# multiplefish/VPLines-SLAM

Measured on AMD Instinct MI355X. Metric: sliding-window BA solves/sec (10 KF, 200 pts + 80 lines, 5 iters), higher is better.
Workload: dtype f64

## Files before the change

### vplines-slam_amd/csrc/ba_step.h

```cpp
#pragma once
#include "ba_common.h"
#include "ba_solve.h"

namespace vpl {

constexpr int SCHUR_THREADS = 256;
constexpr int CHOL_THREADS = 256;
constexpr int BACK_THREADS = 256;

__device__ __forceinline__ void lds_ticket_wait(int* t, int seq) {
  while (__hip_atomic_load(t, __ATOMIC_RELAXED, __HIP_MEMORY_SCOPE_WORKGROUP) != seq) __builtin_amdgcn_s_sleep(1);
  __builtin_amdgcn_fence(__ATOMIC_ACQUIRE, "workgroup", "local");
}
__device__ __forceinline__ void lds_ticket_pass(int* t, int seq, int lane) {
  __builtin_amdgcn_fence(__ATOMIC_RELEASE, "workgroup", "local");
  if (lane == 0) __hip_atomic_store(t, seq + 1, __ATOMIC_RELAXED, __HIP_MEMORY_SCOPE_WORKGROUP);
}

__device__ __forceinline__ int compact2vis(int c, int s, int WS) {
  if (c < WS - 6) { const int v = 6 * s + c; return v < 66 ? v : -1; }
  if (c < WS) return 66 + (c - (WS - 6));
  return c < WS + 2 ? 72 + (c - WS) : -1;
}

// ... 453 lines not shown
      const int k0 = __builtin_amdgcn_readlane(wrow, __builtin_amdgcn_readfirstlane(1 + 3 * ch));
      const int k1 = __builtin_amdgcn_readlane(wrow, __builtin_amdgcn_readfirstlane(2 + 3 * ch));
      const int seq = __builtin_amdgcn_readlane(wrow, __builtin_amdgcn_readfirstlane(3 + 3 * ch));
      nent += k1 - k0;
      if (MIXED && (fetch(k0).x & 64)) {
        SchurWide A;
        A.etab = etab; A.Wp = Wp; A.Wl = Wl; A.WS = WS; A.lC = lC; A.lS = lS; A.lE = lE; A.lG = lG; A.pS = pS; A.pE = pE; A.pG = pG;
        A.Cacc = Cacc; A.tick = tick;
        schur_wide_chunk(A, k0, k1, seq);
        continue;
      }
      double raw0[NTC][4], raw1[NTC][4], raw2[NTC][4];
      constexpr int NPF = 3;
      load_raw(fetch(k0), raw0);
      load_raw(fetch(min(k0 + 1, k1 - 1)), raw1);
      load_raw(fetch(min(k0 + 2, k1 - 1)), raw2);
      const int gcur = fetch(k0).x;
      auto step = [&](int k, double (&rw)[NTC][4]) {
        const int4 e = fetch(k);
#ifdef VPL_STAMPS
        const long long ts0 = __builtin_readcyclecounter();
#endif
        double x[NTC][4];
        transform(e, rw, x);
#ifdef VPL_STAMPS
        const long long ts1 = __builtin_readcyclecounter();
        st_xf += ts1 - ts0;
#endif
        load_raw(fetch(min(k + NPF, k1 - 1)), rw);
#ifdef VPL_STAMPS
        const long long ts2 = __builtin_readcyclecounter();
        st_ld += ts2 - ts1;
#endif
        const bool isl = (e.x & 32) != 0;
#pragma unroll
        for (int a = 0; a < 4; ++a) {
          if (a == 0 || isl) {
            int t = 0;
#pragma unroll
            for (int ta = 0; ta < NTC; ++ta)
#pragma unroll
              for (int tb = 0; tb <= ta; ++tb, ++t) acc[t] = __builtin_amdgcn_mfma_f64_16x16x4f64(x[ta][a], x[tb][a], acc[t], 0, 0, 0);
          }
        }
#ifdef VPL_STAMPS
        st_mf += __builtin_readcyclecounter() - ts2;
#endif
      };
#pragma unroll 1
      for (int kb = k0; kb < k1; kb += NPF) {
        step(kb, raw0);
        if (kb + 1 < k1) step(kb + 1, raw1);
        if (kb + 2 < k1) step(kb + 2, raw2);
      }
      flush(gcur, seq);
    }
#ifdef VPL_STAMPS
    if (lane == 0 && wv < 2) {
      long long* dg_ = B.dbg + (size_t)w * 64 + 30 + 6 * wv;
      dg_[0] = st_xf; dg_[1] = st_ld; dg_[2] = st_mf; dg_[3] = st_flush; dg_[4] = st_wait; dg_[5] = nent;
    }
#endif
  }
  __syncthreads();
  VPL_STAMP(B, w, 3);
  for (int b = tid; b < NV; b += T) qq += 2.0 * Cacc[(NV + 1) * CSQ_LD + b] * uc[vis2cam(b)];
  double* sacc = B.sacc + (size_t)w * SACC_N;
  for (int i = tid; i < SACC_N; i += T) {
    int a, b;
    tri_decode(i, a, b);
    sacc[i] = Cacc[a * CSQ_LD + b];
  }
  a1 = block_sum(a1, red);
  q = block_sum(q, red);
  qq = block_sum(qq, red);
  if (tid == 0) {
    tr->a1 = a1;
    tr->alpha = a1 / (q + qq);
    if (flag[0]) B.path[w] = 2;
  }
  VPL_STAMP(B, w, 4);
}

template <int NTC>
__global__ __launch_bounds__(SCHUR_THREADS, 2) void k_schur(DevBatch B) {
  extern __shared__ double sm[];
  if (blockIdx.x == 0 && threadIdx.x == 0) { B.ord_cnt[2 * ((B.ord_it + 1) & 1)] = 0; B.ord_cnt[2 * ((B.ord_it + 1) & 1) + 1] = 0; }
  schur_body<NTC>(B, ordered_window(B), sm);
}
__global__ __launch_bounds__(SCHUR_THREADS, 2) void k_schur_mixed(DevBatch B) {
  extern __shared__ double sm[];
  if (blockIdx.x == 0 && threadIdx.x == 0) { B.ord_cnt[2 * ((B.ord_it + 1) & 1)] = 0; B.ord_cnt[2 * ((B.ord_it + 1) & 1) + 1] = 0; }
  schur_body<3, true>(B, ordered_window(B), sm);
}
inline size_t schur_smem(int maxP, int maxL, int ntc = 5) {
  const int r1 = std::max(4 * maxP + 28 * maxL, (int)CSQ_N);
  const int maxKS = maxP / 4 + maxL + NF + 2;
  return (size_t)(r1 + 3 * maxP + 22 * maxL + 176 + 24) * sizeof(double) + (size_t)(8 + 4 * maxKS + ntc * (ntc + 1) / 2 * 256) * sizeof(int);
}

constexpr int DN = 90;
constexpr int DNT = 6;
constexpr int DNAP = DNT * (DNT + 1) / 2 * 256;
constexpr int XLD = 80;
constexpr int CHOL_MIN_WAVES = 2;
constexpr int XROWS_A = 36, XROWS_B = 48;
__device__ __forceinline__ constexpr int xcol(int ch, int J) { return ch == 0 ? 16 * (J > 3 ? J - 1 : J) : 16 * (J - 1); }
__device__ __forceinline__ constexpr int tile_row(int t) { return t < 1 ? 0 : t < 3 ? 1 : t < 6 ? 2 : t < 10 ? 3 : t < 15 ? 4 : 5; }

__device__ __forceinline__ int chain_frame(int ch, int b) { return ch == 0 ? 1 + b : 10 - b; }
__device__ __forceinline__ int chain_col(int ch, int b, int lane) {
  if (lane < 18) {
    const int ds = (b & 1) ? 9 : 0;
    const int f = chain_frame(ch, b);
    const int fr = (lane >= ds && lane < ds + 9) ? f : (ch == 0 ? f + 1 : f - 1);
    return 15 * fr + 6 + (lane < 9 ? lane : lane - 9);
  }
  if (ch == 0) {
    if (lane < 27) return 6 + (lane - 18);
    if (lane < 63) return 15 * ((lane - 27) / 6) + (lane - 27) % 6;
    return NC;
  }
  if (lane < 54) return 15 * (5 + (lane - 18) / 6) + (lane - 18) % 6;
  return lane == 54 ? NC : -1;
}
__device__ __forceinline__ int cam2dense(int c) {
  if (c < 0) return -1;
  if (c == NC) return DN;
  const int v = cam2vis(c);
  if (v >= 0) return v;
  if (c < 15) return 72 + (c - 6);
  return (c >= 81 && c < 90) ? c : -1;
}
__device__ __forceinline__ int dense2cam(int d) { return d < NV ? vis2cam(d) : (d < 81 ? 6 + (d - 72) : d); }
__device__ __forceinline__ int chain_dense(int ch, int lane) {
  if (lane < 18) {
    const bool s5 = ch == 0 ? lane < 9 : lane >= 9;
    return s5 ? 81 + (lane < 9 ? lane : lane - 9) : -1;
  }
  return cam2dense(chain_col(ch, 0, lane));
}

__device__ __forceinline__ void chol_body(const DevBatch& B, const int w, double* sm) {
  const int tid = threadIdx.x, T = CHOL_THREADS;
  const int lane = tid & 63, wv = ((tid >> 6) + ((blockIdx.x >> 8) & 1) * 2) & 3;
  TrState* tr = &B.tr[w];
  if (tr->status != 0 || tr->reuse != 0 || B.path[w] != 0) return;
  count_active(B, 1);
  constexpr int REG = (XROWS_A + XROWS_B) * XLD > DNAP ? (XROWS_A + XROWS_B) * XLD : DNAP;
  double* XA = sm;
  double* XBm = sm + XROWS_A * XLD;
  double* S = sm;
  double* scv = sm + REG;
  double* dgv = scv + 176;
  double* ycam = dgv + 176;
  double* yv = ycam + 176;
  double* isd = yv + 96;
  double* Linv = isd + 96;
  double* red = Linv + 256;
  int* flag = (int*)(red + 24);
  double* rsL = (double*)(flag + 8);

  const size_t fb = (size_t)w * B.nfull;
  const double* gscale = B.scale + fb;
  const double* gdiag = B.diag + fb;
  const double* ggrad = B.grad + fb;
  double* ggn = B.gn + fb;
  const double* Hcc = B.Hcc + (size_t)w * NCP;
  const double* gc = B.gc + (size_t)w * NC;
  const double* sacc = B.sacc + (size_t)w * SACC_N;
  const double mu = tr->mu;
  for (int c = tid; c < 176; c += T) { scv[c] = c < NC ? gscale[c] : 0.0; dgv[c] = c < NC ? gdiag[c] : 1.0; ycam[c] = 0.0; }
  if (tid < 4) flag[tid] = 0;
  for (int i = tid; i < (XROWS_A + XROWS_B) * XLD; i += T) sm[i] = 0.0;
  __syncthreads();
  VPL_STAMP(B, w, 8);

  double U[45];
#pragma unroll
  for (int i = 0; i < 45; ++i) U[i] = 0.0;
#define Xs(b, k) U[9 * (b) + (k)]
  if (wv < 2) {
    const int ch = wv, nblk = ch == 0 ? 4 : 5;
    double* Xout = ch == 0 ? XA : XBm;
    const int xd = chain_dense(ch, lane);
    const int xp = xd < 0 ? -1 : xcol(ch, xd >> 4) + (xd & 15);
    bool bad = false;
    auto load_strip = [&](int b, double (&raw)[9]) {
      const int col = chain_col(ch, b, lane);
      const int f = chain_frame(ch, b);
#pragma unroll
      for (int i = 0; i < 9; ++i) {
        const int r = 15 * f + 6 + i;
        raw[i] = 0.0;
        if (col == NC) raw[i] = gc[r];
        else if (col >= 0) raw[i] = Hcc[col > r ? tri(col, r) : tri(r, col)];
      }
    };
    double rawn[9];
    load_strip(0, rawn);
#pragma unroll
    for (int b = 0; b < 5; ++b) {
      if (b < nblk) {
        const int ds = (b & 1) ? 9 : 0, ns = 9 - ds;
        const int col = chain_col(ch, b, lane);
        const int f = chain_frame(ch, b);
        double R[9];
        {
          const double scol = col == NC ? 1.0 : (col >= 0 ? scv[col] : 0.0);
#pragma unroll
          for (int i = 0; i < 9; ++i) {
            const int r = 15 * f + 6 + i;
            R[i] = rawn[i] * (scv[r] * scol);
            if (col == r) R[i] += mu * dgv[r] * dgv[r];
          }
        }
        if (b + 1 < nblk) load_strip(b + 1, rawn);
        if (b > 0) {
          const bool fresh = lane >= ns && lane < ns + 9;
#pragma unroll
          for (int k = 0; k < 9; ++k) {
            const double xk = fresh ? 0.0 : Xs(b - 1, k);
#pragma unroll
            for (int i = 0; i < 9; ++i) R[i] -= readlane_f64(Xs(b - 1, k), ds + i) * xk;
          }
        }
        double piv[9];
#pragma unroll
        for (int k = 0; k < 9; ++k) {
          const double pk = readlane_f64(R[k], ds + k);
          piv[k] = pk;
          if (!(pk > 0.0)) bad = true;
          double rinv = __builtin_amdgcn_rcp(pk);
          rinv = fma(rinv, fma(-pk, rinv, 1.0), rinv);
          rinv = fma(rinv, fma(-pk, rinv, 1.0), rinv);
          const double fj = R[k] * rinv;
#pragma unroll
          for (int i = k + 1; i < 9; ++i) R[i] -= readlane_f64(R[i], ds + k) * fj;
        }
        const bool dcol = cam2dense(col) >= 0;
#pragma unroll
        for (int k = 0; k < 9; ++k) {
          double rs = __builtin_amdgcn_rsq(piv[k]);
          rs = rs * fma(-0.5 * piv[k] * rs, rs, 1.5);
          rs = rs * fma(-0.5 * piv[k] * rs, rs, 1.5);
          if (lane == 0) rsL[(5 * ch + b) * 9 + k] = rs;
          const double xv = R[k] * rs;
          Xs(b, k) = col >= 0 ? xv : 0.0;
          if (xp >= 0) Xout[(9 * b + k) * XLD + xp] = dcol ? xv : 0.0;
        }
        __builtin_amdgcn_fence(__ATOMIC_RELEASE, "workgroup");
        if (lane == 0) __hip_atomic_store(&flag[1 + ch], b + 1, __ATOMIC_RELAXED, __HIP_MEMORY_SCOPE_WORKGROUP);
      }
    }
    if (bad && lane == 0) flag[0] = 1;
  } else {
    const int m = lane & 15, kk = lane >> 4;
    auto h0 = [&](int r, int c) -> double {
      if (r < c) { const int t = r; r = c; c = t; }
      if (r > DN || c == DN) return r == c ? 1.0 : 0.0;
      const int cc = dense2cam(c);
      if (r == DN) return (gc[cc] - (c < NV ? sacc[tri(NV, c)] : 0.0)) * scv[cc];
      const int cr = dense2cam(r);
      double v = Hcc[cr >= cc ? tri(cr, cc) : tri(cc, cr)];
      if (r < NV) v -= sacc[tri(r, c)];
      v *= scv[cr] * scv[cc];
      if (r == c) v += mu * dgv[cr] * dgv[cr];
      return v;
    };
    const int p = __builtin_amdgcn_readfirstlane(wv - 2);
    v4d hs[11], acc[11];
#pragma unroll
    for (int i = 0; i < 11; ++i) acc[i] = v4d{0, 0, 0, 0};
    int have = 0;
#pragma unroll 1
    for (int ks = 0; ks < XROWS_A / 4; ++ks) {
      const int need = min(4, (4 * ks + 3) / 9 + 1);
      while (have < need) {
        have = __hip_atomic_load(&flag[1], __ATOMIC_RELAXED, __HIP_MEMORY_SCOPE_WORKGROUP);
        if (have >= need) __builtin_amdgcn_fence(__ATOMIC_ACQUIRE, "workgroup");
      }
      const double* row = XA + (4 * ks + kk) * XLD + m;
      double x[6];
#pragma unroll
      for (int J = 0; J < 6; ++J) x[J] = J == 3 ? 0.0 : row[xcol(0, J)];
#pragma unroll
      for (int t = 0; t < 21; ++t) {
        const int I = tile_row(t), J = t - I * (I + 1) / 2;
        if ((t & 1) != p || I == 3 || J == 3) continue;
        acc[t >> 1] = __builtin_amdgcn_mfma_f64_16x16x4f64(x[I], x[J], acc[t >> 1], 0, 0, 0);
      }
    }
#pragma unroll
    for (int t = 0; t < 21; ++t) {
      if ((t & 1) != p) continue;
      const int I = tile_row(t), J = t - I * (I + 1) / 2;
      const int r = 16 * I + kk, c = 16 * J + m;
      const v4d h = v4d{h0(r, c), h0(r + 4, c), h0(r + 8, c), h0(r + 12, c)};
      hs[t >> 1] = (I == 3 || J == 3) ? h : h - acc[t >> 1];
      acc[t >> 1] = v4d{0, 0, 0, 0};
    }
    if (p) hs[10] = v4d{0, 0, 0, 0};
    have = 0;
#pragma unroll 1
    for (int ks = 0; ks < XROWS_B / 4; ++ks) {
      const int need = min(5, (4 * ks + 3) / 9 + 1);
      while (have < need) {
        have = __hip_atomic_load(&flag[2], __ATOMIC_RELAXED, __HIP_MEMORY_SCOPE_WORKGROUP);
        if (have >= need) __builtin_amdgcn_fence(__ATOMIC_ACQUIRE, "workgroup");
      }
      const double* row = XBm + (4 * ks + kk) * XLD + m;
      double x[6];
#pragma unroll
      for (int J = 0; J < 6; ++J) x[J] = J == 0 ? 0.0 : row[xcol(1, J)];
#pragma unroll
      for (int t = 0; t < 21; ++t) {
        const int I = tile_row(t), J = t - I * (I + 1) / 2;
        if ((t & 1) != p || J == 0) continue;
        acc[t >> 1] = __builtin_amdgcn_mfma_f64_16x16x4f64(x[I], x[J], acc[t >> 1], 0, 0, 0);
      }
    }
#pragma unroll
    for (int i = 0; i < 11; ++i) {
      const v4d h = hs[i] - acc[i];
      U[4 * i] = h.x; U[4 * i + 1] = h.y; U[4 * i + 2] = h.z; U[4 * i + 3] = h.w;
    }
  }
  __syncthreads();
  VPL_STAMP(B, w, 9);

  if (wv >= 2) {
    const int p = __builtin_amdgcn_readfirstlane(wv - 2);
    const int m = lane & 15, kk = lane >> 4;
#pragma unroll
    for (int t = 0; t < 21; ++t) {
      if ((t & 1) != p) continue;
      double* St = S + (t << 8);
#pragma unroll
// ... 338 lines not shown
```

### vplines-slam_amd/csrc/ba_types.h

```cpp
#pragma once
#include <stdint.h>

namespace vpl {

constexpr int NF = 11;
constexpr int NC = 171;
constexpr int NV = 72;
__host__ __device__ inline int wcol(int c, int s, int WS) {
  if (c >= 66) return WS - 72 + c;
  const int cc = c - 6 * s;
  return (cc >= 0 && cc < WS - 6) ? cc : -1;
}
constexpr int NCP = NC * (NC + 1) / 2;
constexpr int MAXPB = 23;
constexpr int MAXPN = 171;
constexpr int ACT_SLOTS = 64;
constexpr int SK_WSTRIDE = 64;
constexpr int NZ_N = 2628 + 1089 + 1890 + 540;
constexpr int SACC_N = 74 * 75 / 2;
constexpr int MAXKEEP = 80;

__host__ __device__ inline int vis2cam(int v) { return v < 66 ? 15 * (v / 6) + (v % 6) : 165 + (v - 66); }
__host__ __device__ inline int tri(int r, int c) { return r * (r + 1) / 2 + c; }

struct DevOptions {
  int num_iterations, estimate_extrinsic, marginalization_flag, remove_line_outliers;
  double sqrt_info_point, sqrt_info_line, sqrt_info_vp, g_norm, huber_delta;
};

struct DevPreint {
  double sum_dt;
  double dp[3], dq[4] , dv[3], lba[3], lbg[3];
  double dp_dba[9], dp_dbg[9], dq_dbg[9], dv_dba[9], dv_dbg[9];
  double cov[225];
  double sqrt_info[225];
};

struct TrState {
  double radius, mu, x_cost, cand_cost, model_cost_change, x_norm, step_norm, dogleg_step_norm;
  double alpha, a1 , a2 , a3 , initial_cost;
  int iter;
  int status;
  int reuse;
  int step_valid;
  int fresh_lin;
  int num_successful, num_invalid;
  int pad;
};

struct DevBatch {
  int nW;
  int maxP, maxPO, maxL, maxLO;
  int nfull;
  DevOptions opt;

  double *pose, *sb, *ex, *invd, *orth;
  double *pose_c, *sb_c, *ex_c, *invd_c, *orth_c;
  double *lw, *lw_c;
  double *lin_part, *lin_pcost;
  int* lin_flag;
  int ncu;
  double *pose_0, *sb_0, *ex_0, *invd_0, *plk_0;
  double *plk;
  double *gauge;
  int *orth_in;
  double *fail_ref;

  int *nP, *nL;
  int *pt_start, *pt_nobs, *pt_off;
  double *pt_obs;
  int *ps_list, *ps_cnt;
  int *pu_lane, *pu_sub;
  int *pu_cnt, *pu_cnt0;
  int maxPR;
  int prhN;
  int *ln_start, *ln_nobs, *ln_off;
  double *ln_obs;
  int *nLO, *lo_ln;
  int *ll_tab, *ll_np;
  int llNLW, llK, llSlots;
  int *ln_removed;
  int *ln_tri;

  DevPreint *pre;

  int *pr_n, *pr_nb;
  int *pr_kind, *pr_frame, *pr_idx;
  double *pr_x0;
  double *pr_J0, *pr_r0;
  double *pr_H;
  double *pr_g0;
  int prS;
  int *pr_map;

  double *Hcc, *gc;
  int *asm_tab;
  double *Hpp, *gp, *Wp;
  double *Hll, *gl, *Wl;
  int WS, wfill;
  int *order;
  int *ord_cnt;
  int ord_it;
  double *lchol;

  int *sk_tab, *sk_wave;
  int maxKS;
  double *sacc;
  double *ycs;
  double *sx;
  int *path;
  int *nz_tab;

  TrState *tr;
  double *scale, *diag, *grad, *gn;

  int *mg_n, *mg_nb;
  int *mg_kind, *mg_frame, *mg_idx, *mg_cam;
  double *mg_x0;
  double *mg_J0, *mg_r0;
  double *mg_A, *mg_b;
  int *mg_m;
  long long *dbg;
  int *act;
  int launch;
};


struct KeepSrc {
  int nP; const int *pt_start, *pt_nobs;
  int nL; const int *ln_start, *ln_nobs, *ln_removed;
  int pr_nb; const int *pr_kind, *pr_frame;
  bool imu01;
};

__host__ __device__ inline void keep_tables_old(const KeepSrc& S, int* kind, int* frame, int* idx, int* cam, int* n_out,
                                                int* nb_out, int* m_out) {
  bool pose_t[NF], sb_t[NF];
  for (int f = 0; f < NF; ++f) { pose_t[f] = false; sb_t[f] = false; }
  bool ex_t = false, frame0 = false;
  int m = 0;
  for (int p = 0; p < S.nP; ++p)
    if (S.pt_start[p] == 0) { for (int k = 1; k < S.pt_nobs[p]; ++k) pose_t[k] = true; ex_t = frame0 = true; m += 1; }
  for (int l = 0; l < S.nL; ++l)
    if (S.ln_start[l] == 0 && S.ln_nobs[l] >= 2 && !(S.ln_removed && S.ln_removed[l])) {
      for (int k = 1; k < S.ln_nobs[l]; ++k) pose_t[k] = true;
      ex_t = frame0 = true; m += 4;
    }
  for (int b = 0; b < S.pr_nb; ++b) {
    if (S.pr_kind[b] == 0) pose_t[S.pr_frame[b]] = true;
    else if (S.pr_kind[b] == 1) sb_t[S.pr_frame[b]] = true;
    else ex_t = true;
  }
  if (S.imu01) { pose_t[0] = pose_t[1] = true; sb_t[0] = sb_t[1] = true; }
  int nb = 0, n = 0;
  for (int f = 1; f < NF; ++f) if (pose_t[f]) { kind[nb] = 0; frame[nb] = f - 1; idx[nb] = n; cam[nb] = 15 * f; n += 6; ++nb; }
  for (int f = 1; f < NF; ++f) if (sb_t[f]) { kind[nb] = 1; frame[nb] = f - 1; idx[nb] = n; cam[nb] = 15 * f + 6; n += 9; ++nb; }
  if (ex_t) { kind[nb] = 2; frame[nb] = 0; idx[nb] = n; cam[nb] = 165; n += 6; ++nb; }
  *n_out = n; *nb_out = nb;
  *m_out = m + ((pose_t[0] || frame0) ? 6 : 0) + (sb_t[0] ? 9 : 0);
}

__host__ __device__ inline int keep_tables_second_new(int pr_nb, const int* pr_kind, const int* pr_frame, int* kind,
                                                       int* frame, int* idx, int* cam, int* n_out, int* nb_out) {
  bool has = false;
  for (int b = 0; b < pr_nb; ++b) {
    if (pr_kind[b] == 0 && pr_frame[b] == NF - 2) has = true;
    if (pr_kind[b] == 1 && pr_frame[b] == NF - 2) return -1;
  }
  *n_out = 0; *nb_out = 0;
  if (!has) return 0;
  int nb = 0, n = 0;
  for (int k = 0; k < 3; ++k)
    for (int f = 0; f < NF; ++f)
      for (int b = 0; b < pr_nb; ++b) {
        if (pr_kind[b] != k || (k < 2 && pr_frame[b] != f) || (k == 2 && f != 0)) continue;
        if (k == 0 && f == NF - 2) continue;
        kind[nb] = k; frame[nb] = (k < 2 && f == NF - 1) ? NF - 2 : (k == 2 ? 0 : f); idx[nb] = n;
        cam[nb] = k == 0 ? 15 * f : (k == 1 ? 15 * f + 6 : 165);
        n += k == 1 ? 9 : 6; ++nb;
      }
  *n_out = n; *nb_out = nb;
  return 1;
}

}
```

### vplines-slam_amd/csrc/vplines_ba.hip

```cpp
#include <hip/hip_runtime.h>

#include <algorithm>
#include <chrono>
#include <memory>
#include <cmath>
#include <cstdio>
#include <cstdlib>
#include <cstring>
#include <functional>
#include <map>
#include <string>
#include <vector>

#include "vplines_ba.h"
#include "ba_types.h"
#include "ba_lin.h"
#include "ba_pack.h"
#include "ba_solve.h"
#include "ba_step.h"
#include "ba_marg.h"
#include "ba_prior_eig.h"
#include "ba_lineopt.h"
#include "ba_factors.h"
#include "ba_odo.h"
// ... 243 lines not shown
  hipError_t alloc(size_t bytes) { return hipMalloc(&p, bytes ? bytes : 8); }
  double* d() { return (double*)p; }
};

template <typename Launch>
static int eval_generic(vpl_ctx* c, int n, const double* params, int psz, const double* consts, int csz, int nres,
                        int njac, double* residuals, double* jac, Launch launch) {
  if (!c || n < 0 || !params || !consts || !residuals) return VPL_E_INVALID;
  if (n == 0) return VPL_OK;
  HIPCHK(c, hipSetDevice(c->device));
  DevBuf dp, dc, dr, dj;
  HIPCHK(c, dp.alloc((size_t)n * psz * 8));
  HIPCHK(c, dc.alloc((size_t)n * csz * 8));
  HIPCHK(c, dr.alloc((size_t)n * nres * 8));
  if (jac) HIPCHK(c, dj.alloc((size_t)n * njac * 8));
  HIPCHK(c, hipMemcpyAsync(dp.p, params, (size_t)n * psz * 8, hipMemcpyHostToDevice, c->stream));
  HIPCHK(c, hipMemcpyAsync(dc.p, consts, (size_t)n * csz * 8, hipMemcpyHostToDevice, c->stream));
  launch(dp.d(), dc.d(), dr.d(), jac ? dj.d() : nullptr);
  HIPCHK(c, hipGetLastError());
  HIPCHK(c, hipMemcpyAsync(residuals, dr.p, (size_t)n * nres * 8, hipMemcpyDeviceToHost, c->stream));
  if (jac) HIPCHK(c, hipMemcpyAsync(jac, dj.p, (size_t)n * njac * 8, hipMemcpyDeviceToHost, c->stream));
  HIPCHK(c, hipStreamSynchronize(c->stream));
  return VPL_OK;
}

template <typename Keep>
static void scatter_lines(const vpl_ctx* c, size_t w, vpl_window& v, const double* plk, Keep keep) {
  const std::vector<int>& lmap = c->h_lmap[w];
  for (size_t dl = 0; dl < lmap.size(); ++dl)
    if (keep((int)dl, lmap[dl])) std::memcpy(v.line_plk + (size_t)lmap[dl] * 6, plk + dl * 6, 6 * 8);
}
static int scatter_solved_lines(const vpl_ctx* c, size_t w, vpl_window& v, const double* plk, const int* removed) {
  if (v.line_removed) std::fill(v.line_removed, v.line_removed + v.n_lines, 0);
  int n = 0;
  scatter_lines(c, w, v, plk, [&](int dl, int l) {
    if (v.line_removed) v.line_removed[l] = removed[dl] ? 1 : 0;
    n += removed[dl] ? 1 : 0;
    return !removed[dl];
  });
  return n;
}
static void fill_report(vpl_solve_report& r, const TrState& t) {
  std::memset(&r, 0, sizeof(r));
  r.iterations = t.iter;
  r.num_successful_steps = t.num_successful;
  r.termination = t.status == 1 ? 1 : t.status == 2 ? 2 : 0;
  r.initial_cost = t.initial_cost;
  r.final_cost = t.x_cost;
}

extern "C" {

void vpl_ba_default_options(vpl_ba_options* o) {
  o->num_iterations = 5;
  o->estimate_extrinsic = 1;
  o->marginalization_flag = VPL_MARGIN_OLD;
  o->remove_line_outliers = 0;
  o->focal_length = 460.0;
  o->line_factor = 306.666666667;
  o->vp_factor = 10.0;
  o->g_norm = 9.81007;
  o->acc_n = 0.08; o->gyr_n = 0.004; o->acc_w = 0.00004; o->gyr_w = 2.0e-6;
  o->huber_delta = 1.0;
}

static int ctx_init(vpl_ctx* c, int device, int max_windows, int max_points, int max_point_obs, int max_lines, int max_line_obs) {
  { const char* g = getenv("VPL_DEBUG_GUARDS"); c->guards = g && g[0] == '1'; }
  c->device = device;
  c->maxW = max_windows;
  c->maxP = max_points > 0 ? (max_points + 1) & ~1 : 2;
  c->maxPO = max_point_obs > 0 ? max_point_obs : 1;
  c->maxL = max_lines > 0 ? max_lines : 1;
  c->maxLO = max_line_obs > 0 ? max_line_obs : 1;
  if (2 * c->maxP + 18 * c->maxL > NAP - 2 * CROWS * CW) return VPL_E_CAPACITY;
  if (4 * c->maxP + 28 * c->maxL > 2 * CROWS * CW) return VPL_E_CAPACITY;
  if (solve_smem(c->maxP, c->maxL) > 159 * 1024) return VPL_E_CAPACITY;
  DevBatch& B = c->B;
  std::memset(&B, 0, sizeof(B));
  B.maxP = c->maxP; B.maxPO = c->maxPO; B.maxL = c->maxL; B.maxLO = c->maxLO;
  B.nfull = NC + B.maxP + 4 * B.maxL;
  {
    int ncu = 0;
    if (hipDeviceGetAttribute(&ncu, hipDeviceAttributeMultiprocessorCount, device) != hipSuccess || ncu <= 0) ncu = 256;
    if (const char* sv = std::getenv("VPL_BA_LIN_SPLIT")) ncu = std::atoi(sv) ? 1 << 30 : 0;
    B.ncu = ncu;
  }
  B.maxPR = max_point_unit_rounds(B.maxP, B.maxPO);
  B.maxKS = max_schur_ksteps(B.maxP, B.maxL);
  B.llSlots = line_lane_slots(B.maxL);
  const size_t W = max_windows;
  hipError_t e = hipSuccess;
#define AL(ptr, n) if (e == hipSuccess) e = dalloc(c, &B.ptr, (size_t)(n))
  AL(pose, W * 77); AL(sb, W * 99); AL(ex, W * 7); AL(invd, W * B.maxP); AL(orth, W * B.maxL * 4);
  AL(pose_c, W * 77); AL(sb_c, W * 99); AL(ex_c, W * 7); AL(invd_c, W * B.maxP); AL(orth_c, W * B.maxL * 4); AL(lw, W * B.maxL * 6); AL(lw_c, W * B.maxL * 6);
  AL(lin_part, W * LIN_PART); AL(lin_pcost, W); AL(lin_flag, W);
  AL(pose_0, W * 77); AL(sb_0, W * 99); AL(ex_0, W * 7); AL(invd_0, W * B.maxP); AL(plk_0, W * B.maxL * 6);
  AL(plk, W * B.maxL * 6); AL(gauge, W * 4); AL(fail_ref, W * 13); AL(orth_in, W);
  AL(nP, W); AL(nL, W);
  AL(pt_start, W * B.maxP); AL(pt_nobs, W * B.maxP); AL(pt_off, W * B.maxP); AL(pt_obs, W * B.maxPO * 3);
  AL(ps_list, W * B.maxP); AL(ps_cnt, W * (NF + 1)); AL(pu_lane, W * B.maxPR * 1024); AL(pu_sub, W * B.maxPR * 512); AL(pu_cnt, W); AL(pu_cnt0, W);
  AL(ln_start, W * B.maxL); AL(ln_nobs, W * B.maxL); AL(ln_off, W * B.maxL); AL(ln_obs, W * B.maxLO * 8);
  AL(nLO, W); AL(lo_ln, W * B.maxLO);
  AL(ll_tab, W * B.llSlots * 2); AL(ll_np, W);
  AL(pre, W * NF);
  AL(pr_n, W); AL(pr_nb, W); AL(pr_kind, W * MAXPB); AL(pr_frame, W * MAXPB); AL(pr_idx, W * MAXPB);
  AL(pr_x0, W * MAXPB * 9); AL(pr_J0, W * MAXPN * MAXPN); AL(pr_r0, W * MAXPN); AL(pr_H, W * MAXPN * MAXPN); AL(pr_g0, W * MAXPN);
  AL(pr_map, W * MAXPN);
  AL(Hcc, W * NCP); AL(gc, W * NC); AL(asm_tab, 2 * NCP); AL(Hpp, W * B.maxP); AL(gp, W * B.maxP); AL(Wp, W * B.maxP * NV);
  AL(Hll, W * B.maxL * 16); AL(gl, W * B.maxL * 4); AL(Wl, W * B.maxL * 4 * NV); AL(lchol, W * B.maxL * 10);
  AL(tr, W);
  AL(scale, W * B.nfull); AL(diag, W * B.nfull); AL(grad, W * B.nfull); AL(gn, W * B.nfull);
  AL(mg_n, W); AL(mg_nb, W); AL(mg_kind, W * MAXPB); AL(mg_frame, W * MAXPB); AL(mg_idx, W * MAXPB);
  AL(mg_cam, W * MAXPB); AL(mg_x0, W * MAXPB * 9); AL(mg_J0, W * MAXKEEP * MAXKEEP); AL(mg_r0, W * MAXKEEP);
  AL(mg_A, W * MAXKEEP * MAXKEEP); AL(mg_b, W * MAXKEEP); AL(mg_m, W); AL(dbg, W * 64); AL(ln_removed, W * B.maxL); AL(ln_tri, W * B.maxL);
  if (e == hipSuccess) e = dalloc(c, &c->d_act, (size_t)ACT_SLOTS * 4);
  AL(order, 2 * W); AL(ord_cnt, 4);
  AL(sk_tab, W * B.maxKS * 4); AL(sk_wave, W * 8 * SK_WSTRIDE); AL(sacc, W * SACC_N); AL(nz_tab, NZ_N); AL(ycs, W * 176); AL(sx, W * 8); AL(path, W);
#undef AL
  if (e != hipSuccess) return VPL_E_HIP;
  if (lin_smem_base(c->maxP, c->maxL) > LIN_LDS_BUDGET) return VPL_E_CAPACITY;
  B.prhN = lin_prh_n(c->maxP, c->maxL);
  {
    std::vector<int> tab(2 * NCP);
    for (int r = 0, e2 = 0; r < NC; ++r)
      for (int cc = 0; cc <= r; ++cc, ++e2) lin_asm_entry(r, cc, &tab[2 * e2]);
    if (hipMemcpy(B.asm_tab, tab.data(), tab.size() * sizeof(int), hipMemcpyHostToDevice) != hipSuccess) return VPL_E_HIP;
  }
  {
    std::vector<int> nz;
    for (int r = 0; r < NC; ++r)
      for (int cc = 0; cc <= r; ++cc) {
        const bool vis = cam2vis(r) >= 0 && cam2vis(cc) >= 0;
        const int fr = r < 165 ? r / 15 : -1, fc = cc < 165 ? cc / 15 : -1;
        const bool band = fr >= 0 && fc >= 0 && (fr == fc || fr == fc + 1);
        const bool sb0 = cc >= 6 && cc < 15 && cam2vis(r) >= 0;
        if (vis || band || sb0) nz.push_back(tri(r, cc) | r << 14 | cc << 22);
      }
    if ((int)nz.size() != NZ_N || hipMemcpy(B.nz_tab, nz.data(), nz.size() * sizeof(int), hipMemcpyHostToDevice) != hipSuccess) return VPL_E_HIP;
  }
  static size_t lin_max = 0, solve_max = 0, schur_max = 0, back_max = 0;
  lin_max = std::max(lin_max, lin_smem(c->maxP, c->maxL));
  solve_max = std::max(solve_max, solve_smem(c->maxP, c->maxL));
  schur_max = std::max(schur_max, schur_smem(c->maxP, c->maxL));
  back_max = std::max(back_max, back_smem(c->maxP, c->maxL));
  if (schur_max > 159 * 1024 || back_max > 159 * 1024) return VPL_E_CAPACITY;
  const std::pair<const void*, size_t> lds[] = {
      {(const void*)k_lin2, lin_max}, {(const void*)k_lin<1>, lin_max}, {(const void*)k_lin<2>, lin_max},
      {(const void*)k_solve, solve_max}, {(const void*)k_schur<3>, schur_max}, {(const void*)k_schur<5>, schur_max},
      {(const void*)k_schur_mixed, schur_max}, {(const void*)k_chol, CHOL_SMEM}, {(const void*)k_back, back_max},
      {(const void*)k_prep, PREP_SMEM}, {(const void*)k_marg<MARG_THREADS>, 159 * 1024}, {(const void*)k_marg<256>, MARG_LDS_SMALL},
      {(const void*)k_prior_eigen, prior_eig_layout(MAXKEEP).bytes}};
  for (const auto& k : lds)
    if (hipFuncSetAttribute(k.first, hipFuncAttributeMaxDynamicSharedMemorySize, (int)k.second) != hipSuccess) return VPL_E_HIP;
  vpl_ba_default_options(&c->opt);
  if (const char* gv = std::getenv("VPL_BA_GRAPH")) c->use_graph = std::atoi(gv) != 0;
  if (const char* gv = std::getenv("VPL_BA_GENERAL")) c->force_general = std::atoi(gv) != 0;
  if (const char* gv = std::getenv("VPL_BA_SCHUR_WIDE")) { c->schur_wide_all = std::atoi(gv) > 0; c->schur_never_wide = std::atoi(gv) < 0; }
  return VPL_OK;
}

int vpl_ctx_create(vpl_ctx** out, int device, int max_windows, int max_points, int max_point_obs, int max_lines,
                   int max_line_obs) {
  if (!out || max_windows < 1 || max_points < 0 || max_lines < 0) return VPL_E_INVALID;
  int ndev = 0;
  if (hipGetDeviceCount(&ndev) != hipSuccess || ndev == 0 || device >= ndev) return VPL_E_NODEVICE;
  if (hipSetDevice(device) != hipSuccess) return VPL_E_NODEVICE;
  vpl_ctx* c = new vpl_ctx();
  const int rc = ctx_init(c, device, max_windows, max_points, max_point_obs, max_lines, max_line_obs);
  if (rc != VPL_OK) {
    free_arrays(c);
    delete c;
    return rc;
  }
  *out = c;
  return VPL_OK;
}

void vpl_ctx_destroy(vpl_ctx* c) {
  if (!c) return;
  (void)hipSetDevice(c->device);
  (void)hipDeviceSynchronize();
  drop_graph(c);
  free_arrays(c);
  c->stage.release();
  for (hipEvent_t& e : c->leg_ev) if (e) (void)hipEventDestroy(e);
  delete c;
}

int vpl_ctx_set_stream(vpl_ctx* c, void* s) {
  if (!c) return VPL_E_INVALID;
  const int rs = settle(c);
  if (rs) return rs;
  if (c->stream != (hipStream_t)s) {
    HIPCHK(c, hipSetDevice(c->device));
    (void)hipStreamSynchronize(c->stream);
    (void)hipGetLastError();
  }
  drop_graph(c);
  c->stream = (hipStream_t)s;
  return VPL_OK;
// ... 870 lines not shown
      for (int k = 0; k < nLns; ++k) std::memcpy(win[job->lw[k]].line_plk + 6 * job->lidx[k], &job->ld[(size_t)k * 6], 48);
    }
    for (int w = 0; w < nW; ++w) {
      std::memmove(win[w].pose[0], win[w].pose[1], sizeof(win[w].pose[0]) * WS);
      std::memmove(win[w].speed_bias[0], win[w].speed_bias[1], sizeof(win[w].speed_bias[0]) * WS);
    }
    return VPL_OK;
  });
}
int vpl_ba_slide_window(vpl_ctx* c, int nW, vpl_window* win, int flag, double init_depth, vpl_slide_tracks* out) {
  return slide_window_impl(c, nW, win, flag, init_depth, out, false);
}
int vpl_ba_slide_window_async(vpl_ctx* c, int nW, vpl_window* win, int flag, double init_depth, vpl_slide_tracks* out) {
  return slide_window_impl(c, nW, win, flag, init_depth, out, true);
}

static void launch_line_opt(vpl_ctx* c, int nW) {
  DevBatch B = c->B;
  B.opt.marginalization_flag = VPL_MARGIN_NONE;
  B.opt.remove_line_outliers = 1;
  const dim3 grid(nW);
  hipStream_t s = c->stream;
  launch_prep(c, B, nW, s);
  {
    KTimer t(c, "k_line_opt");
    if (4 * c->maxL <= LOPT_THREADS) hipLaunchKernelGGL(k_line_opt<4>, grid, dim3(LOPT_THREADS), 0, s, B);
    else if (2 * c->maxL <= LOPT_THREADS) hipLaunchKernelGGL(k_line_opt<2>, grid, dim3(LOPT_THREADS), 0, s, B);
    else hipLaunchKernelGGL(k_line_opt<1>, grid, dim3(LOPT_THREADS), 0, s, B);
  }
  { KTimer t(c, "k_gauge"); hipLaunchKernelGGL(k_gauge, grid, dim3(128), 0, s, B); }
}
static int only_line_opt_impl(vpl_ctx* c, int nW, vpl_window* win, const vpl_ba_options* opt_in, vpl_solve_report* reports, bool async,
                              const vpl_ba_options* solve_opt = nullptr) {
  if (!c || !win || !opt_in || nW < 1) return VPL_E_INVALID;
  if (c->maxL > LOPT_THREADS) return fail(c, VPL_E_CAPACITY, "onlyLineOpt handles at most 256 lines per window");
  vpl_ba_options opt = *opt_in;
  opt.marginalization_flag = VPL_MARGIN_NONE;
  opt.remove_line_outliers = 1;
  int rc = upload_impl(c, nW, win, solve_opt ? solve_opt : &opt, false);
  if (rc) return rc;
  const DevBatch& B = c->B;
  hipStream_t s = c->stream;
  launch_line_opt(c, nW);
  HIPCHK(c, hipGetLastError());
  const size_t W = nW;
  auto plk = std::make_shared<std::vector<double>>(W * B.maxL * 6);
  auto removed = std::make_shared<std::vector<int>>(W * B.maxL);
  auto tr = std::make_shared<std::vector<TrState>>(W);
  HIPCHK(c, hipMemcpyAsync(plk->data(), B.plk, plk->size() * 8, hipMemcpyDeviceToHost, s));
  HIPCHK(c, hipMemcpyAsync(removed->data(), B.ln_removed, removed->size() * 4, hipMemcpyDeviceToHost, s));
  HIPCHK(c, hipMemcpyAsync(tr->data(), B.tr, W * sizeof(TrState), hipMemcpyDeviceToHost, s));
  const int maxL = B.maxL;
  return finish_or_defer(c, async, [c, win, reports, W, plk, removed, tr, maxL, s]() -> int {
    HIPCHK(c, hipStreamSynchronize(s));
    for (size_t w = 0; w < W; ++w) {
      vpl_window& v = win[w];
      if (reports) std::memset(&reports[w], 0, sizeof(reports[w]));
      if (c->h_lmap[w].size() < 4) {
        if (v.line_removed) std::fill(v.line_removed, v.line_removed + v.n_lines, 0);
        continue;
      }
      const int nrem = scatter_solved_lines(c, w, v, &(*plk)[w * maxL * 6], &(*removed)[w * maxL]);
      if (reports) {
        fill_report(reports[w], (*tr)[w]);
        reports[w].n_lines_removed = nrem;
      }
    }
    return VPL_OK;
  });
}
int vpl_ba_only_line_opt(vpl_ctx* c, int nW, vpl_window* win, const vpl_ba_options* opt, vpl_solve_report* reports) {
  return only_line_opt_impl(c, nW, win, opt, reports, false);
}
int vpl_ba_only_line_opt_async(vpl_ctx* c, int nW, vpl_window* win, const vpl_ba_options* opt, vpl_solve_report* reports) {
  return only_line_opt_impl(c, nW, win, opt, reports, true);
}

static void launch_solve(vpl_ctx* c, int w0, int nw, hipStream_t s) {
  DevBatch B = c->B;
  B.ord_it = 0;
  B.act = c->timing ? c->d_act : nullptr;
  B.launch = 0;
  if (c->timing) { c->ltimes.clear(); (void)hipMemsetAsync(c->d_act, 0, sizeof(int) * ACT_SLOTS * 4, s); }
  const dim3 grid(nw);
  launch_prep(c, B, nw, s);
  ++B.launch;
  { KTimer t(c, "k_lin"); hipLaunchKernelGGL(k_lin2, dim3(16 * ((nw + 7) / 8)), dim3(LIN_THREADS), lin_smem(c->maxP, c->maxL), s, B); }
  ++B.launch;
  for (int it = 0; it < c->opt.num_iterations; ++it) {
    B.ord_it = it;
    { KTimer t(c, "k_schur");
      if (B.WS + 2 <= 48) hipLaunchKernelGGL(k_schur<3>, grid, dim3(SCHUR_THREADS), schur_smem(B.maxP, B.maxL, 3), s, B);
      else if (c->schur_wide_all || (c->schur_mostly_wide && !c->schur_never_wide)) hipLaunchKernelGGL(k_schur<5>, grid, dim3(SCHUR_THREADS), schur_smem(B.maxP, B.maxL, 5), s, B);
      else hipLaunchKernelGGL(k_schur_mixed, grid, dim3(SCHUR_THREADS), schur_smem(B.maxP, B.maxL, 3), s, B); }
    ++B.launch;
    { KTimer t(c, "k_chol"); hipLaunchKernelGGL(k_chol, grid, dim3(CHOL_THREADS), CHOL_SMEM, s, B); }
    ++B.launch;
    { KTimer t(c, "k_solve"); hipLaunchKernelGGL(k_solve, grid, dim3(SOLVE_THREADS), solve_smem(B.maxP, B.maxL), s, B); }
    ++B.launch;
    { KTimer t(c, "k_back"); hipLaunchKernelGGL(k_back, grid, dim3(BACK_THREADS), back_smem(B.maxP, B.maxL), s, B); }
    ++B.launch;
    { KTimer t(c, "k_cost"); hipLaunchKernelGGL(k_cost, grid, dim3(COST_THREADS), 0, s, B); }
    ++B.launch;
    if (it + 1 < c->opt.num_iterations) {
      B.ord_it = it + 1;
      KTimer t(c, "k_lin");
      hipLaunchKernelGGL(k_lin2, dim3(16 * ((nw + 7) / 8)), dim3(LIN_THREADS), lin_smem(c->maxP, c->maxL), s, B);
    }
    if (it + 1 < c->opt.num_iterations) ++B.launch;
  }
  B.ord_it = 0;
  { KTimer t(c, "k_gauge"); hipLaunchKernelGGL(k_gauge, grid, dim3(128), 0, s, B); }
  ++B.launch;
  launch_marg(c, B, nw, s);
}

int vpl_ba_solve(vpl_ctx* c) {
  if (c) { const int rs = settle(c); if (rs) return rs; }
  if (!c || c->nW < 1) return VPL_E_INVALID;
  HIPCHK(c, hipSetDevice(c->device));
  if (c->opt.marginalization_flag != VPL_MARGIN_NONE) { c->prior_resident = true; c->prior_resident_nW = c->nW; }
  if (c->leg_timing) {
    HIPCHK(c, hipEventRecord(c->leg_ev[2], c->stream));
    launch_solve(c, 0, c->nW, c->stream);
    HIPCHK(c, hipGetLastError());
    HIPCHK(c, hipEventRecord(c->leg_ev[3], c->stream));
    return VPL_OK;
  }
  if (c->use_graph && !c->timing && c->stream != nullptr) {
    if (!c->graph_exec) {
      hipGraph_t graph = nullptr;
      HIPCHK(c, hipStreamBeginCapture(c->stream, hipStreamCaptureModeThreadLocal));
      launch_solve(c, 0, c->nW, c->stream);
      HIPCHK(c, hipStreamEndCapture(c->stream, &graph));
      hipError_t e = hipGraphInstantiate(&c->graph_exec, graph, nullptr, nullptr, 0);
      (void)hipGraphDestroy(graph);
      if (e != hipSuccess) { c->graph_exec = nullptr; return fail(c, VPL_E_HIP, std::string("hipGraphInstantiate: ") + hipGetErrorString(e)); }
    }
    HIPCHK(c, hipGraphLaunch(c->graph_exec, c->stream));
    return VPL_OK;
  }
  launch_solve(c, 0, c->nW, c->stream);
  HIPCHK(c, hipGetLastError());
  return VPL_OK;
}

struct PriorFetch {
  Span<int> mg_n, mg_nb, mg_kind, mg_frame, mg_idx, mg_m;
  Span<double> mg_x0, mg_r0;
  std::vector<Span<double>> J0;
};
static void prior_fetch_plan(vpl_ctx* c, int nW, PriorFetch& F, Stage& S) {
  const DevBatch& B = c->B;
  const size_t W = nW;
  F.mg_m = S.take<int>(W); F.mg_n = S.take<int>(W); F.mg_nb = S.take<int>(W);
  F.mg_kind = S.take<int>(W * MAXPB); F.mg_frame = S.take<int>(W * MAXPB); F.mg_idx = S.take<int>(W * MAXPB);
  F.mg_x0 = S.take<double>(W * MAXPB * 9); F.mg_r0 = S.take<double>(W * MAXKEEP);
  S.from_device(F.mg_m.p, B.mg_m, W); S.from_device(F.mg_n.p, B.mg_n, W); S.from_device(F.mg_nb.p, B.mg_nb, W);
  S.from_device(F.mg_kind.p, B.mg_kind, W * MAXPB); S.from_device(F.mg_frame.p, B.mg_frame, W * MAXPB);
  S.from_device(F.mg_idx.p, B.mg_idx, W * MAXPB);
  S.from_device(F.mg_x0.p, B.mg_x0, W * MAXPB * 9); S.from_device(F.mg_r0.p, B.mg_r0, W * MAXKEEP);
  F.J0.resize(W);
  for (size_t w = 0; w < W; ++w) {
    const int n = w < c->h_mg_n.size() ? std::min(std::max(c->h_mg_n[w], 0), (int)MAXKEEP) : (int)MAXKEEP;
    F.J0[w] = S.take<double>((size_t)n * n);
    S.from_device(F.J0[w].p, B.mg_J0 + w * (size_t)MAXKEEP * MAXKEEP, (size_t)n * n);
  }
}
static int prior_fetch_finish(vpl_ctx* c, int nW, const PriorFetch& F, vpl_prior* priors, std::vector<int>& mn) {
  DevBatch& B = c->B;
  const size_t W = nW;
  const Span<int>&mg_n = F.mg_n, &mg_nb = F.mg_nb, &mg_kind = F.mg_kind, &mg_frame = F.mg_frame, &mg_idx = F.mg_idx, &mg_m = F.mg_m;
  const Span<double>& mg_x0 = F.mg_x0, &mg_r0 = F.mg_r0;
  mn.assign(2 * W, 0);
  for (size_t w = 0; w < W; ++w) {
    mn[2 * w] = mg_m[w];
    if (c->h_passthrough[w] >= 0) {
// ... 844 lines not shown
```

Measured before the change: 258,400.

## Precompute chain elimination in helper blocks during the Schur kernel

Doubles the Schur kernel grid so that the extra blocks run the banded chain elimination, which depends only on Hcc/gc and the scaling, concurrently with the Schur complement. Results go to a global handoff buffer. The Cholesky kernel then loads the precomputed chain factors instead of doing the serial elimination itself, shortening its critical path. Helper blocks recompute scale and diag locally on the first iteration. They are only used when the number of windows being factored is at most half the CU count, so idle CUs are used without oversubscribing. The cost is extra global traffic and more blocks per Schur launch.

```diff
diff --git a/vplines-slam_amd/csrc/ba_step.h b/vplines-slam_amd/csrc/ba_step.h
--- a/vplines-slam_amd/csrc/ba_step.h
+++ b/vplines-slam_amd/csrc/ba_step.h
@@ -559,14 +559,17 @@
   VPL_STAMP(B, w, 4);
 }
 
+__device__ __forceinline__ void chain_helper_block(const DevBatch& B, double* sm);
 template <int NTC>
 __global__ __launch_bounds__(SCHUR_THREADS, 2) void k_schur(DevBatch B) {
   extern __shared__ double sm[];
+  if ((int)blockIdx.x >= B.nW) { chain_helper_block(B, sm); return; }
   if (blockIdx.x == 0 && threadIdx.x == 0) { B.ord_cnt[2 * ((B.ord_it + 1) & 1)] = 0; B.ord_cnt[2 * ((B.ord_it + 1) & 1) + 1] = 0; }
   schur_body<NTC>(B, ordered_window(B), sm);
 }
 __global__ __launch_bounds__(SCHUR_THREADS, 2) void k_schur_mixed(DevBatch B) {
   extern __shared__ double sm[];
+  if ((int)blockIdx.x >= B.nW) { chain_helper_block(B, sm); return; }
   if (blockIdx.x == 0 && threadIdx.x == 0) { B.ord_cnt[2 * ((B.ord_it + 1) & 1)] = 0; B.ord_cnt[2 * ((B.ord_it + 1) & 1) + 1] = 0; }
   schur_body<3, true>(B, ordered_window(B), sm);
 }
@@ -616,6 +619,137 @@
     return s5 ? 81 + (lane < 9 ? lane : lane - 9) : -1;
   }
   return cam2dense(chain_col(ch, 0, lane));
+}
+
+#define Xs(b, k) U[9 * (b) + (k)]
+template <bool TO_LDS>
+__device__ __forceinline__ bool chain_eliminate(const int ch, const int lane, const double* Hcc, const double* gc, const double* scv,
+                                                const double* dgv, const double mu, double (&U)[45], double* rsL, double* Xout,
+                                                int* progress) {
+  const int nblk = ch == 0 ? 4 : 5;
+  const int xd = chain_dense(ch, lane);
+  const int xp = xd < 0 ? -1 : xcol(ch, xd >> 4) + (xd & 15);
+  bool bad = false;
+  auto load_strip = [&](int b, double (&raw)[9]) {
+    const int col = chain_col(ch, b, lane);
+    const int f = chain_frame(ch, b);
+#pragma unroll
+    for (int i = 0; i < 9; ++i) {
+      const int r = 15 * f + 6 + i;
+      raw[i] = 0.0;
+      if (col == NC) raw[i] = gc[r];
+      else if (col >= 0) raw[i] = Hcc[col > r ? tri(col, r) : tri(r, col)];
+    }
+  };
+  double rawn[9];
+  load_strip(0, rawn);
+#pragma unroll
+  for (int b = 0; b < 5; ++b) {
+    if (b < nblk) {
+      const int ds = (b & 1) ? 9 : 0, ns = 9 - ds;
+      const int col = chain_col(ch, b, lane);
+      const int f = chain_frame(ch, b);
+      double R[9];
+      {
+        const double scol = col == NC ? 1.0 : (col >= 0 ? scv[col] : 0.0);
+#pragma unroll
+        for (int i = 0; i < 9; ++i) {
+          const int r = 15 * f + 6 + i;
+          R[i] = rawn[i] * (scv[r] * scol);
+          if (col == r) R[i] += mu * dgv[r] * dgv[r];
+        }
+      }
+      if (b + 1 < nblk) load_strip(b + 1, rawn);
+      if (b > 0) {
+        const bool fresh = lane >= ns && lane < ns + 9;
+#pragma unroll
+        for (int k = 0; k < 9; ++k) {
+          const double xk = fresh ? 0.0 : Xs(b - 1, k);
+#pragma unroll
+          for (int i = 0; i < 9; ++i) R[i] -= readlane_f64(Xs(b - 1, k), ds + i) * xk;
+        }
+      }
+      double piv[9];
+#pragma unroll
+      for (int k = 0; k < 9; ++k) {
+        const double pk = readlane_f64(R[k], ds + k);
+        piv[k] = pk;
+        if (!(pk > 0.0)) bad = true;
+        double rinv = __builtin_amdgcn_rcp(pk);
+        rinv = fma(rinv, fma(-pk, rinv, 1.0), rinv);
+        rinv = fma(rinv, fma(-pk, rinv, 1.0), rinv);
+        const double fj = R[k] * rinv;
+#pragma unroll
+        for (int i = k + 1; i < 9; ++i) R[i] -= readlane_f64(R[i], ds + k) * fj;
+      }
+      const bool dcol = cam2dense(col) >= 0;
+#pragma unroll
+      for (int k = 0; k < 9; ++k) {
+        double rs = __builtin_amdgcn_rsq(piv[k]);
+        rs = rs * fma(-0.5 * piv[k] * rs, rs, 1.5);
+        rs = rs * fma(-0.5 * piv[k] * rs, rs, 1.5);
+        if (lane == 0) rsL[(5 * ch + b) * 9 + k] = rs;
+        const double xv = R[k] * rs;
+        Xs(b, k) = col >= 0 ? xv : 0.0;
+        if (TO_LDS && xp >= 0) Xout[(9 * b + k) * XLD + xp] = dcol ? xv : 0.0;
+      }
+      if (TO_LDS) {
+        __builtin_amdgcn_fence(__ATOMIC_RELEASE, "workgroup");
+        if (lane == 0) __hip_atomic_store(progress, b + 1, __ATOMIC_RELAXED, __HIP_MEMORY_SCOPE_WORKGROUP);
+      }
+    }
+  }
+  return bad;
+}
+#undef Xs
+
+__device__ __forceinline__ void chain_helper_block(const DevBatch& B, double* sm) {
+  const int tid = threadIdx.x, T = SCHUR_THREADS;
+  const int lane = tid & 63, wv = tid >> 6;
+  const int pos = (int)blockIdx.x - B.nW;
+  const int w = __builtin_amdgcn_readfirstlane(B.ord_it == 0 ? pos : B.order[(size_t)(B.ord_it & 1) * B.nW + pos]);
+  double* hand = B.chain + (size_t)w * CHAIN_HAND_N;
+  int* hflag = (int*)(hand + CHAIN_HAND_RS + 90);
+  const TrState* tr = &B.tr[w];
+  const int nfactor = B.ord_it == 0 ? B.nW : B.ord_cnt[2 * (B.ord_it & 1)];
+  const bool work = nfactor <= B.chain_limit && tr->status == 0 && tr->reuse == 0 && B.path[w] == 0;
+  if (!__builtin_amdgcn_readfirstlane((int)work)) {
+    if (tid == 0) hflag[0] = 0;
+    return;
+  }
+  VPL_STAMP(B, w, 56);
+  double* scv = sm;
+  double* dgv = scv + 176;
+  const double* gscale = B.scale + (size_t)w * B.nfull;
+  const double* Hcc = B.Hcc + (size_t)w * NCP;
+  const double* gc = B.gc + (size_t)w * NC;
+  const double mu = tr->mu;
+  const bool first = (tr->iter == 0);
+  for (int c = tid; c < 176; c += T) {
+    double s = 0.0, d = 1.0;
+    if (c < NC) {
+      const double h = Hcc[tri(c, c)];
+      s = first ? 1.0 / (1.0 + sqrt(h)) : gscale[c];
+      d = sqrt(fmin(fmax(s * s * h, kMinDiag), kMaxDiag));
+    }
+    scv[c] = s; dgv[c] = d;
+  }
+  __syncthreads();
+  VPL_STAMP(B, w, 57);
+  if (wv < 2) {
+    const int ch = wv, nrow = ch == 0 ? CHAIN_ROWS_A : CHAIN_ROWS_B;
+    double U[45];
+#pragma unroll
+    for (int i = 0; i < 45; ++i) U[i] = 0.0;
+    const bool bad = chain_eliminate<false>(ch, lane, Hcc, gc, scv, dgv, mu, U, hand + CHAIN_HAND_RS, nullptr, nullptr);
+    double* hx = hand + (ch == 0 ? 0 : CHAIN_ROWS_A * 64) + lane;
+#pragma unroll
+    for (int i = 0; i < 45; ++i)
+      if (i < nrow) hx[i * 64] = U[i];
+    if (lane == 0) hflag[1 + ch] = bad ? 1 : 0;
+  }
+  if (tid == 0) hflag[0] = 1;
+  VPL_STAMP(B, w, 58);
 }
 
 __device__ __forceinline__ void chol_body(const DevBatch& B, const int w, double* sm) {
@@ -647,6 +781,9 @@
   const double* gc = B.gc + (size_t)w * NC;
   const double* sacc = B.sacc + (size_t)w * SACC_N;
   const double mu = tr->mu;
+  const double* hand = B.chain + (size_t)w * CHAIN_HAND_N;
+  const int* hflag = (const int*)(hand + CHAIN_HAND_RS + 90);
+  const int handed_ld = hflag[0];
   for (int c = tid; c < 176; c += T) { scv[c] = c < NC ? gscale[c] : 0.0; dgv[c] = c < NC ? gdiag[c] : 1.0; ycam[c] = 0.0; }
   if (tid < 4) flag[tid] = 0;
   for (int i = tid; i < (XROWS_A + XROWS_B) * XLD; i += T) sm[i] = 0.0;
@@ -657,80 +794,35 @@
 #pragma unroll
   for (int i = 0; i < 45; ++i) U[i] = 0.0;
 #define Xs(b, k) U[9 * (b) + (k)]
+  const int handed = __builtin_amdgcn_readfirstlane(handed_ld);
   if (wv < 2) {
-    const int ch = wv, nblk = ch == 0 ? 4 : 5;
+    const int ch = wv;
     double* Xout = ch == 0 ? XA : XBm;
-    const int xd = chain_dense(ch, lane);
-    const int xp = xd < 0 ? -1 : xcol(ch, xd >> 4) + (xd & 15);
-    bool bad = false;
-    auto load_strip = [&](int b, double (&raw)[9]) {
-      const int col = chain_col(ch, b, lane);
-      const int f = chain_frame(ch, b);
-#pragma unroll
-      for (int i = 0; i < 9; ++i) {
-        const int r = 15 * f + 6 + i;
-        raw[i] = 0.0;
-        if (col == NC) raw[i] = gc[r];
-        else if (col >= 0) raw[i] = Hcc[col > r ? tri(col, r) : tri(r, col)];
-      }
-    };
-    double rawn[9];
-    load_strip(0, rawn);
-#pragma unroll
-    for (int b = 0; b < 5; ++b) {
-      if (b < nblk) {
-        const int ds = (b & 1) ? 9 : 0, ns = 9 - ds;
-        const int col = chain_col(ch, b, lane);
-        const int f = chain_frame(ch, b);
-        double R[9];
-        {
-          const double scol = col == NC ? 1.0 : (col >= 0 ? scv[col] : 0.0);
-#pragma unroll
-          for (int i = 0; i < 9; ++i) {
-            const int r = 15 * f + 6 + i;
-            R[i] = rawn[i] * (scv[r] * scol);
-            if (col == r) R[i] += mu * dgv[r] * dgv[r];
-          }
-        }
-        if (b + 1 < nblk) load_strip(b + 1, rawn);
-        if (b > 0) {
-          const bool fresh = lane >= ns && lane < ns + 9;
-#pragma unroll
-          for (int k = 0; k < 9; ++k) {
-            const double xk = fresh ? 0.0 : Xs(b - 1, k);
-#pragma unroll
-            for (int i = 0; i < 9; ++i) R[i] -= readlane_f64(Xs(b - 1, k), ds + i) * xk;
-          }
-        }
-        double piv[9];
-#pragma unroll
-        for (int k = 0; k < 9; ++k) {
-          const double pk = readlane_f64(R[k], ds + k);
-          piv[k] = pk;
-          if (!(pk > 0.0)) bad = true;
-          double rinv = __builtin_amdgcn_rcp(pk);
-          rinv = fma(rinv, fma(-pk, rinv, 1.0), rinv);
-          rinv = fma(rinv, fma(-pk, rinv, 1.0), rinv);
-          const double fj = R[k] * rinv;
-#pragma unroll
-          for (int i = k + 1; i < 9; ++i) R[i] -= readlane_f64(R[i], ds + k) * fj;
-        }
-        const bool dcol = cam2dense(col) >= 0;
-#pragma unroll
-        for (int k = 0; k < 9; ++k) {
-          double rs = __builtin_amdgcn_rsq(piv[k]);
-          rs = rs * fma(-0.5 * piv[k] * rs, rs, 1.5);
-          rs = rs * fma(-0.5 * piv[k] * rs, rs, 1.5);
-          if (lane == 0) rsL[(5 * ch + b) * 9 + k] = rs;
-          const double xv = R[k] * rs;
-          Xs(b, k) = col >= 0 ? xv : 0.0;
-          if (xp >= 0) Xout[(9 * b + k) * XLD + xp] = dcol ? xv : 0.0;
-        }
-        __builtin_amdgcn_fence(__ATOMIC_RELEASE, "workgroup");
-        if (lane == 0) __hip_atomic_store(&flag[1 + ch], b + 1, __ATOMIC_RELAXED, __HIP_MEMORY_SCOPE_WORKGROUP);
-      }
-    }
-    if (bad && lane == 0) flag[0] = 1;
+    if (handed) {
+      const int nblk = ch == 0 ? 4 : 5;
+      const double* hx = hand + (ch == 0 ? 0 : CHAIN_ROWS_A * 64) + lane;
+#pragma unroll
+      for (int i = 0; i < 45; ++i)
+        if (i < 9 * nblk) U[i] = hx[i * 64];
+      if (lane < 45) rsL[45 * ch + lane] = hand[CHAIN_HAND_RS + 45 * ch + lane];
+      const int xd = chain_dense(ch, lane);
+      const int xp = xd < 0 ? -1 : xcol(ch, xd >> 4) + (xd & 15);
+#pragma unroll
+      for (int b = 0; b < 5; ++b) {
+        if (b < nblk) {
+          const bool dcol = cam2dense(chain_col(ch, b, lane)) >= 0;
+#pragma unroll
+          for (int k = 0; k < 9; ++k)
+            if (xp >= 0) Xout[(9 * b + k) * XLD + xp] = dcol ? Xs(b, k) : 0.0;
+        }
+      }
+      if (lane == 0 && hflag[1 + ch]) flag[0] = 1;
+      __builtin_amdgcn_fence(__ATOMIC_RELEASE, "workgroup");
+      if (lane == 0) __hip_atomic_store(&flag[1 + ch], nblk, __ATOMIC_RELAXED, __HIP_MEMORY_SCOPE_WORKGROUP);
+    } else {
+      const bool bad = chain_eliminate<true>(ch, lane, Hcc, gc, scv, dgv, mu, U, rsL, Xout, &flag[1 + ch]);
+      if (bad && lane == 0) flag[0] = 1;
+    }
   } else {
     const int m = lane & 15, kk = lane >> 4;
     auto h0 = [&](int r, int c) -> double {
diff --git a/vplines-slam_amd/csrc/ba_types.h b/vplines-slam_amd/csrc/ba_types.h
--- a/vplines-slam_amd/csrc/ba_types.h
+++ b/vplines-slam_amd/csrc/ba_types.h
@@ -18,6 +18,9 @@
 constexpr int SK_WSTRIDE = 64;
 constexpr int NZ_N = 2628 + 1089 + 1890 + 540;
 constexpr int SACC_N = 74 * 75 / 2;
+constexpr int CHAIN_ROWS_A = 36, CHAIN_ROWS_B = 45;
+constexpr int CHAIN_HAND_RS = (CHAIN_ROWS_A + CHAIN_ROWS_B) * 64;
+constexpr int CHAIN_HAND_N = CHAIN_HAND_RS + 90 + 2;
 constexpr int MAXKEEP = 80;
 
 __host__ __device__ inline int vis2cam(int v) { return v < 66 ? 15 * (v / 6) + (v % 6) : 165 + (v - 66); }
@@ -108,6 +111,8 @@
   double *sacc;
   double *ycs;
   double *sx;
+  double *chain;
+  int chain_limit;
   int *path;
   int *nz_tab;
 
diff --git a/vplines-slam_amd/csrc/vplines_ba.hip b/vplines-slam_amd/csrc/vplines_ba.hip
--- a/vplines-slam_amd/csrc/vplines_ba.hip
+++ b/vplines-slam_amd/csrc/vplines_ba.hip
@@ -349,6 +349,11 @@
   {
     int ncu = 0;
     if (hipDeviceGetAttribute(&ncu, hipDeviceAttributeMultiprocessorCount, device) != hipSuccess || ncu <= 0) ncu = 256;
+    B.chain_limit = ncu / 2;
+    if (const char* sv = std::getenv("VPL_BA_CHAIN_SPLIT")) {
+      const int n = std::atoi(sv);
+      B.chain_limit = n == 1 ? 1 << 30 : std::max(n, 0);
+    }
     if (const char* sv = std::getenv("VPL_BA_LIN_SPLIT")) ncu = std::atoi(sv) ? 1 << 30 : 0;
     B.ncu = ncu;
   }
@@ -382,7 +387,7 @@
   AL(mg_A, W * MAXKEEP * MAXKEEP); AL(mg_b, W * MAXKEEP); AL(mg_m, W); AL(dbg, W * 64); AL(ln_removed, W * B.maxL); AL(ln_tri, W * B.maxL);
   if (e == hipSuccess) e = dalloc(c, &c->d_act, (size_t)ACT_SLOTS * 4);
   AL(order, 2 * W); AL(ord_cnt, 4);
-  AL(sk_tab, W * B.maxKS * 4); AL(sk_wave, W * 8 * SK_WSTRIDE); AL(sacc, W * SACC_N); AL(nz_tab, NZ_N); AL(ycs, W * 176); AL(sx, W * 8); AL(path, W);
+  AL(sk_tab, W * B.maxKS * 4); AL(sk_wave, W * 8 * SK_WSTRIDE); AL(sacc, W * SACC_N); AL(nz_tab, NZ_N); AL(ycs, W * 176); AL(sx, W * 8); AL(path, W); AL(chain, W * CHAIN_HAND_N);
 #undef AL
   if (e != hipSuccess) return VPL_E_HIP;
   if (lin_smem_base(c->maxP, c->maxL) > LIN_LDS_BUDGET) return VPL_E_CAPACITY;
@@ -1419,7 +1424,7 @@
   B.act = c->timing ? c->d_act : nullptr;
   B.launch = 0;
   if (c->timing) { c->ltimes.clear(); (void)hipMemsetAsync(c->d_act, 0, sizeof(int) * ACT_SLOTS * 4, s); }
-  const dim3 grid(nw);
+  const dim3 grid(nw), grid2(2 * nw);
   launch_prep(c, B, nw, s);
   ++B.launch;
   { KTimer t(c, "k_lin"); hipLaunchKernelGGL(k_lin2, dim3(16 * ((nw + 7) / 8)), dim3(LIN_THREADS), lin_smem(c->maxP, c->maxL), s, B); }
@@ -1427,9 +1432,9 @@
   for (int it = 0; it < c->opt.num_iterations; ++it) {
     B.ord_it = it;
     { KTimer t(c, "k_schur");
-      if (B.WS + 2 <= 48) hipLaunchKernelGGL(k_schur<3>, grid, dim3(SCHUR_THREADS), schur_smem(B.maxP, B.maxL, 3), s, B);
-      else if (c->schur_wide_all || (c->schur_mostly_wide && !c->schur_never_wide)) hipLaunchKernelGGL(k_schur<5>, grid, dim3(SCHUR_THREADS), schur_smem(B.maxP, B.maxL, 5), s, B);
-      else hipLaunchKernelGGL(k_schur_mixed, grid, dim3(SCHUR_THREADS), schur_smem(B.maxP, B.maxL, 3), s, B); }
+      if (B.WS + 2 <= 48) hipLaunchKernelGGL(k_schur<3>, grid2, dim3(SCHUR_THREADS), schur_smem(B.maxP, B.maxL, 3), s, B);
+      else if (c->schur_wide_all || (c->schur_mostly_wide && !c->schur_never_wide)) hipLaunchKernelGGL(k_schur<5>, grid2, dim3(SCHUR_THREADS), schur_smem(B.maxP, B.maxL, 5), s, B);
+      else hipLaunchKernelGGL(k_schur_mixed, grid2, dim3(SCHUR_THREADS), schur_smem(B.maxP, B.maxL, 3), s, B); }
     ++B.launch;
     { KTimer t(c, "k_chol"); hipLaunchKernelGGL(k_chol, grid, dim3(CHOL_THREADS), CHOL_SMEM, s, B); }
     ++B.launch;
```

New measurement: 257,800. No clear change (-0.2%).
